# YooSungHyun/RNNTransducer

Measured on AMD Instinct MI355X. Metric: utterances/sec, higher is better.
Workload: dtype f32

## Files before the change

### include/rnnt_hip.h

```cpp
#ifndef RNNT_HIP_H_
#define RNNT_HIP_H_

#include <stddef.h>
#include <stdint.h>

#ifdef __cplusplus
extern "C" {
#endif

#define RNNT_HIP_ABI_VERSION 4

#define RNNT_OK 0
#define RNNT_ERR_INVALID (-1)
#define RNNT_ERR_LAUNCH (-2)
#define RNNT_ERR_UNSUPPORTED (-3)
#define RNNT_ERR_TIMEOUT (-4)

int rnnt_hip_version(void);
const char* rnnt_hip_last_error(void);
int rnnt_hip_device_cus(void);

enum {
  RNNT_K_GEMM = 0,
  RNNT_K_LSTM_FWD = 1,
// ... 24 lines not shown
  const float* A;
  int64_t a_div, a_so, a_si, a_sk;
  int32_t a_mc;
  const int64_t* a_rowidx;
  const float* B;
  int64_t b_sn, b_sk;
  float* C;
  int64_t c_div, c_so, c_si;
  const float* bias;
  const float* aux;
  uint32_t flags;
  void* workspace;
  size_t workspace_bytes;
} rnnt_gemm_desc;

size_t rnnt_hip_gemm_workspace_bytes(int64_t M, int64_t N, int64_t K);
int rnnt_hip_gemm_f32(const rnnt_gemm_desc* d, void* stream);

size_t rnnt_hip_hp_bytes(int64_t rows, int64_t K);
int rnnt_hip_hp_split(const float* x, int64_t rows, int64_t K, int64_t ld, int32_t transpose, int64_t src_rows, int64_t shift,
                      void* planes, uint32_t* amax, int32_t amax_given, void* stream);
int rnnt_hip_hp_split_both(const float* x, int64_t M, int64_t C, int64_t ld, const uint32_t* rowmax, const uint32_t* colmax,
                           void* planes_rm, void* planes_t, void* stream);
size_t rnnt_hip_gemm_hp_workspace_bytes(int64_t M, int64_t N, int64_t K);
int rnnt_hip_gemm_hp(const void* A, const uint32_t* a_amax, const void* B, const uint32_t* b_amax, int64_t M, int64_t N, int64_t K,
                     float* C, int64_t ldc, const float* bias, uint32_t flags, void* workspace, size_t workspace_bytes,
                     void* stream);

typedef struct rnnt_hp_problem {
  const void* A; const uint32_t* a_amax;
  const void* B; const uint32_t* b_amax;
  int64_t M, N, K;
  float* C; int64_t ldc;
  uint32_t flags;
} rnnt_hp_problem;
size_t rnnt_hip_gemm_hp_grouped_workspace_bytes(const rnnt_hp_problem* problems, int32_t n);
int rnnt_hip_gemm_hp_grouped(const rnnt_hp_problem* problems, int32_t n, uint32_t xcd_skip, void* workspace, size_t workspace_bytes,
                             void* stream);

#define RNNT_CELL_LSTM 0
#define RNNT_CELL_GRU 1
#define RNNT_CELL_RNN_TANH 2
#define RNNT_CELL_RNN_RELU 3

typedef struct rnnt_lstm_desc {
  int32_t T, B, I, H, D;
// ... 273 lines not shown
```

### rnntransducer_amd/_lib.py

```python
from __future__ import annotations

import ctypes as C
import os

_HERE = os.path.dirname(os.path.abspath(__file__))
LIB_PATH = os.environ.get("RNNT_HIP_LIB") or os.path.join(_HERE, "csrc", "librnnt_hip.so")
ABI_VERSION = 4

GEMM_GELU_A, GEMM_GELU_B, GEMM_ACCUM, GEMM_MUL_DGELU, GEMM_EXACT_F32 = 1, 2, 4, 8, 16
GEMM_HP_F16 = 32
PRECISION_FP32, PRECISION_F16 = 0, 1
CELL_LSTM, CELL_GRU, CELL_RNN_TANH, CELL_RNN_RELU = 0, 1, 2, 3

c_f32p = C.c_void_p
c_i64 = C.c_int64
c_i32 = C.c_int32


class GemmDesc(C.Structure):
    _fields_ = [("M", c_i64), ("N", c_i64), ("K", c_i64), ("A", C.c_void_p), ("a_div", c_i64), ("a_so", c_i64),
                ("a_si", c_i64), ("a_sk", c_i64), ("a_mc", c_i32), ("a_rowidx", C.c_void_p), ("B", C.c_void_p),
                ("b_sn", c_i64), ("b_sk", c_i64), ("C", C.c_void_p), ("c_div", c_i64), ("c_so", c_i64),
                ("c_si", c_i64), ("bias", C.c_void_p), ("aux", C.c_void_p), ("flags", C.c_uint32),
                ("workspace", C.c_void_p), ("workspace_bytes", C.c_size_t)]
# ... 85 lines not shown
                ("blank", c_i32), ("beam", c_i32), ("improved", c_i32), ("state_beam", C.c_double), ("expand_beam", C.c_double),
                ("max_candidates", c_i32), ("max_pops", c_i32), ("max_states", c_i32), ("max_nodes", c_i32), ("max_len", c_i32),
                ("A", C.c_void_p), ("lens", C.c_void_p), ("emb", C.c_void_p),
                ("w_ih", C.c_void_p * DECODE_MAX_LAYERS), ("w_hh", C.c_void_p * DECODE_MAX_LAYERS),
                ("b_ih", C.c_void_p * DECODE_MAX_LAYERS), ("b_hh", C.c_void_p * DECODE_MAX_LAYERS),
                ("w_o", C.c_void_p), ("b_o", C.c_void_p), ("w_d", C.c_void_p), ("ld_d", c_i64),
                ("workspace", C.c_void_p), ("workspace_bytes", C.c_size_t), ("tokens", C.c_void_p), ("out_lens", C.c_void_p),
                ("scores", C.c_void_p), ("count", C.c_void_p), ("status", C.c_void_p), ("commit", C.c_void_p),
                ("ncommit", C.c_void_p), ("stats", C.c_void_p)]


SYMBOLS = {
    "rnnt_hip_version": (C.c_int, []),
    "rnnt_hip_last_error": (C.c_char_p, []),
    "rnnt_hip_device_cus": (C.c_int, []),
    "rnnt_hip_prof_enable": (C.c_int, [C.c_int]),
    "rnnt_hip_prof_collect": (C.c_int, [C.c_void_p, C.c_void_p, C.c_void_p, C.c_int]),
    "rnnt_hip_lstm_launch_log_enable": (C.c_int, [C.c_int]),
    "rnnt_hip_lstm_launch_log": (c_i64, [C.c_char_p, C.c_size_t]),
    "rnnt_hip_gemm_workspace_bytes": (C.c_size_t, [c_i64, c_i64, c_i64]),
    "rnnt_hip_gemm_f32": (C.c_int, [C.POINTER(GemmDesc), C.c_void_p]),
    "rnnt_hip_hp_bytes": (C.c_size_t, [c_i64, c_i64]),
    "rnnt_hip_hp_split": (C.c_int, [C.c_void_p, c_i64, c_i64, c_i64, c_i32, c_i64, c_i64, C.c_void_p, C.c_void_p, c_i32, C.c_void_p]),
    "rnnt_hip_gemm_hp_workspace_bytes": (C.c_size_t, [c_i64, c_i64, c_i64]),
    "rnnt_hip_gemm_hp": (C.c_int, [C.c_void_p, C.c_void_p, C.c_void_p, C.c_void_p, c_i64, c_i64, c_i64, C.c_void_p, c_i64, C.c_void_p,
                                  C.c_uint32, C.c_void_p, C.c_size_t, C.c_void_p]),
    "rnnt_hip_hp_split_both": (C.c_int, [C.c_void_p, c_i64, c_i64, c_i64, C.c_void_p, C.c_void_p, C.c_void_p, C.c_void_p, C.c_void_p]),
    "rnnt_hip_gemm_hp_grouped_workspace_bytes": (C.c_size_t, [C.POINTER(HpProblem), c_i32]),
    "rnnt_hip_gemm_hp_grouped": (C.c_int, [C.POINTER(HpProblem), c_i32, C.c_uint32, C.c_void_p, C.c_size_t, C.c_void_p]),
    "rnnt_hip_lstm_workspace_bytes": (C.c_size_t, [c_i32] * 5),
    "rnnt_hip_lstm_max_batch": (c_i32, [c_i32, c_i32, c_i32]),
    "rnnt_hip_lstm_free_xcds": (c_i32, [c_i32] * 5),
    "rnnt_hip_lstm_takes_row_idx": (c_i32, [c_i32] * 6),
    "rnnt_hip_lstm_fwd": (C.c_int, [C.POINTER(LstmDesc), C.c_void_p]),
    "rnnt_hip_lstm_fwd_ex": (C.c_int, [C.POINTER(LstmDesc), C.c_uint32, C.c_void_p]),
    "rnnt_hip_lstm_takes_f16": (c_i32, [c_i32] * 6),
    "rnnt_hip_lstm_bwd": (C.c_int, [C.POINTER(LstmBwdDesc), C.c_void_p]),
    "rnnt_hip_lstm_bwd_ex": (C.c_int, [C.POINTER(LstmBwdDesc), C.c_uint32, C.c_void_p]),
    "rnnt_hip_lstm_check": (C.c_int, [C.c_void_p, C.c_void_p]),
    "rnnt_hip_lstm_debug_read": (C.c_int, [C.c_void_p, c_i32, c_i32, c_i32, c_i32, c_i32, C.c_void_p, c_i32, C.c_void_p]),
    "rnnt_hip_joint_loss_workspace_bytes": (C.c_size_t, [c_i32] * 4),
    "rnnt_hip_joint_loss_fwd_bwd": (C.c_int, [C.c_void_p, c_i64, c_i64, C.c_void_p, c_i64, c_i64, C.c_void_p, C.c_void_p,
                                               C.c_void_p, C.c_void_p, c_i32, c_i32, c_i32, c_i32, c_i32, C.c_float,
                                               C.c_void_p, C.c_void_p, C.c_void_p, C.c_void_p, C.c_size_t, C.c_void_p]),
    "rnnt_hip_joint_loss_bwd": (C.c_int, [C.c_void_p, c_i64, c_i64, C.c_void_p, c_i64, c_i64, C.c_void_p, C.c_void_p,
                                           C.c_void_p, C.c_void_p, c_i32, c_i32, c_i32, c_i32, c_i32, C.c_float, C.c_void_p, c_i32,
# ... 71 lines not shown
```

### rnntransducer_amd/csrc/common.hpp

```cpp
#pragma once
#include <hip/hip_runtime.h>
#include <stdarg.h>
#include <stdint.h>
#include <stdio.h>

#include <atomic>

#include "rnnt_hip.h"

namespace rnnt {

void set_error(const char* fmt, ...);

#define RNNT_CHECK_ARG(cond, ...)      \
  do {                                 \
    if (!(cond)) {                     \
      ::rnnt::set_error(__VA_ARGS__);  \
      return RNNT_ERR_INVALID;         \
    }                                  \
  } while (0)

#define RNNT_CHECK_HIP(expr)                                                          \
  do {                                                                                \
    hipError_t e_ = (expr);                                                           \
// ... 4 lines not shown
  } while (0)

#define RNNT_CHECK_LAUNCH() RNNT_CHECK_HIP(hipGetLastError())

struct ProfScope {
  ProfScope(int kind, double work, hipStream_t s);
  ~ProfScope();
  int kind_;
  double work_;
  hipStream_t stream_;
  void* start_;
};

extern std::atomic<bool> g_launch_log_on;
void launch_log_note(const void* kernel, hipStream_t s);

static inline int64_t ceil_div(int64_t a, int64_t b) { return (a + b - 1) / b; }

size_t hp_plane_bytes(int64_t rows, int64_t K);
int hp_colmax(const float* x, int64_t rows, int64_t C, int64_t ld, uint32_t* amax, hipStream_t s);
int hp_split(const float* x, int64_t rows, int64_t K, int64_t ld, uint32_t* amax, void* planes, hipStream_t s, const int* rowidx = nullptr);
int hp_split_t(const float* x, int64_t R, int64_t K, int64_t ld, int64_t Ksrc, int64_t shift, const uint32_t* amax, void* planes,
               hipStream_t s, const int* kidx = nullptr);
int hp_split_both(const float* x, int64_t M, int64_t C, int64_t ld, const uint32_t* rowmax, const uint32_t* colmax, void* planes_rm,
                  void* planes_t, hipStream_t s, const int* rowidx = nullptr);
size_t hp_gemm_workspace_bytes(int64_t M, int64_t N, int64_t K);
int hp_gemm(const void* A, const uint32_t* a_amax, const void* B, const uint32_t* b_amax, int64_t M, int64_t N, int64_t K, float* C,
            int64_t c_div, int64_t c_so, int64_t c_si, const float* bias, unsigned flags, void* workspace, size_t workspace_bytes,
            hipStream_t s, const int* a_rowidx = nullptr, int64_t a_plane_rows = 0, const int* c_rowidx = nullptr);
struct HpProblem {
  const void* A; const uint32_t* a_amax; const void* B; const uint32_t* b_amax;
  int64_t M, N, K;
  float* C; int64_t ldc;
  unsigned flags;
};
constexpr int HP_GROUP_MAX = 4;
size_t hp_gemm_grouped_workspace_bytes(const int64_t* MN, int n);
int hp_gemm_grouped(const HpProblem* pr, int n, unsigned xcd_skip, unsigned* counter, void* workspace, size_t workspace_bytes,
                    hipStream_t s, unsigned* status = nullptr);
constexpr size_t HPQ_HEADER_BYTES = 256;
static inline size_t align_up(size_t a, size_t b) { return (a + b - 1) / b * b; }

__device__ __forceinline__ float gelu_tanh(float x) {
  const float k0 = 0.7978845608028654f, k1 = 0.044715f;
  float u = k0 * (x + k1 * x * x * x);
  return 0.5f * x * (1.0f + tanhf(u));
// ... 51 lines not shown
```

### rnntransducer_amd/csrc/gemm_hp.hip

```cpp
#include "common.hpp"

#include <stdlib.h>

namespace rnnt {
namespace {

typedef _Float16 f16x8 __attribute__((ext_vector_type(8)));
typedef __attribute__((address_space(3))) void lds_void;

constexpr int HP_BM = 256, HP_BN = 256, HP_BK = 32;
constexpr int HP_STAGE = (HP_BM + HP_BN) * 128;
constexpr int HP_RSRC = 0x00027000;

__device__ __forceinline__ float hp_scale_from_amax(unsigned amax_bits) {
  int eb = (int)((amax_bits >> 23) & 255u);
  if (eb == 0) return 1.0f;
  eb = eb < 15 ? 15 : eb;
  return __uint_as_float((unsigned)(268 - eb) << 23);
}
__device__ __forceinline__ float hp_inv_scale_from_amax(unsigned amax_bits) {
  int eb = (int)((amax_bits >> 23) & 255u);
  if (eb == 0) return 1.0f;
  eb = eb < 15 ? 15 : eb;
  return __uint_as_float((unsigned)(eb - 14) << 23);
}

__global__ void __launch_bounds__(256) hp_colmax_kernel(const float* __restrict__ x, long rows, int C, long ld, long rows_per_chunk,
                                                        unsigned* __restrict__ out) {
  const int c = blockIdx.x * 256 + threadIdx.x;
  if (c >= C) return;
  const long r0 = (long)blockIdx.y * rows_per_chunk, r1 = min(rows, r0 + rows_per_chunk);
  unsigned m = 0;
  for (long r = r0; r < r1; ++r) m = max(m, __float_as_uint(x[r * ld + c]) & 0x7fffffffu);
  if (m != 0) atomicMax(out + c, m);
}

__device__ __forceinline__ void hp_split8(const float (&x)[8], float scale, u32x4& hi, u32x4& lo) {
  f16x8 h, l;
#pragma unroll
  for (int e = 0; e < 8; ++e) {
    const float v = x[e] * scale;
    const _Float16 a = (_Float16)v;
    h[e] = a;
    l[e] = (_Float16)(v - (float)a);
  }
  hi = __builtin_bit_cast(u32x4, h);
  lo = __builtin_bit_cast(u32x4, l);
}

__global__ void __launch_bounds__(256) hp_split_kernel(const float* __restrict__ x, long rows, int K, long ld, unsigned* __restrict__ amax,
                                                       char* __restrict__ out, const int* __restrict__ rowidx) {
  const int Kp = (K + 31) & ~31, cpr = Kp >> 3;
  const int lane = threadIdx.x & 63;
  const bool vec = (ld & 3) == 0 && (reinterpret_cast<uintptr_t>(x) & 15) == 0;
  for (long ri = (long)blockIdx.x * 4 + (threadIdx.x >> 6); ri < rows; ri += (long)gridDim.x * 4) {
    const long r = rowidx ? (long)rowidx[ri] : ri;
    const float* row = x + r * ld;
// ... 13 lines not shown
#pragma unroll
    for (int o = 32; o > 0; o >>= 1) m = max(m, (unsigned)__shfl_xor((int)m, o));
    if (lane == 0) amax[r] = m;
    const float scale = hp_scale_from_amax(m);
    for (int c = lane; c < cpr; c += 64) {
      const int k = 8 * c;
      float v[8];
      if (vec && k + 7 < K) {
        const f32x4 a = *reinterpret_cast<const f32x4*>(row + k), b = *reinterpret_cast<const f32x4*>(row + k + 4);
        v[0] = a[0]; v[1] = a[1]; v[2] = a[2]; v[3] = a[3]; v[4] = b[0]; v[5] = b[1]; v[6] = b[2]; v[7] = b[3];
      } else {
#pragma unroll
        for (int e = 0; e < 8; ++e) v[e] = (k + e < K) ? row[k + e] : 0.f;
      }
      u32x4 hi, lo;
      hp_split8(v, scale, hi, lo);
      char* dst = out + (r * (Kp >> 5) + (c >> 2)) * 128 + 16 * (c & 3);
      *reinterpret_cast<u32x4*>(dst) = hi;
      *reinterpret_cast<u32x4*>(dst + 64) = lo;
    }
  }
}

__global__ void __launch_bounds__(256) hp_split_t_kernel(const float* __restrict__ x, int R, int K, long ld, int Ksrc, int shift,
                                                         const unsigned* __restrict__ amax, char* __restrict__ out,
                                                         const int* __restrict__ kidx) {
  __shared__ float tile[32][257];
  const int kb = blockIdx.x, r0 = blockIdx.y * 256;
  const int tid = threadIdx.x;
  const bool vec = (ld & 3) == 0 && (reinterpret_cast<uintptr_t>(x) & 15) == 0;
#pragma unroll
  for (int q = 0; q < 8; ++q) {
    const int kk = 4 * q + (tid >> 6);
    const int kdst = kb * 32 + kk;
    const int ksrc = (kidx ? (kdst < K ? kidx[kdst] : 0) : kdst) + shift;
    const int c = 4 * (tid & 63);
    f32x4 v = {0.f, 0.f, 0.f, 0.f};
    if (kdst < K && ksrc >= 0 && ksrc < Ksrc) {
      const float* src = x + (long)ksrc * ld + r0 + c;
      if (vec && r0 + c + 3 < R) {
        v = *reinterpret_cast<const f32x4*>(src);
      } else {
#pragma unroll
        for (int e = 0; e < 4; ++e)
          if (r0 + c + e < R) v[e] = src[e];
      }
    }
#pragma unroll
    for (int e = 0; e < 4; ++e) tile[kk][c + e] = v[e];
  }
  __syncthreads();
  const int Kp32 = (K + 31) >> 5;
#pragma unroll
  for (int ps = 0; ps < 4; ++ps) {
    const int rl = (tid >> 2) + 64 * ps, ch = tid & 3;
    if (r0 + rl < R) {
      float v[8];
#pragma unroll
      for (int e = 0; e < 8; ++e) v[e] = tile[8 * ch + e][rl];
      u32x4 hi, lo;
      hp_split8(v, hp_scale_from_amax(amax[r0 + rl]), hi, lo);
      char* dst = out + ((long)(r0 + rl) * Kp32 + kb) * 128 + 16 * ch;
// ... 285 lines not shown
    counter[9] = 1u;
    if (status) __hip_atomic_store(status, 2u, __ATOMIC_RELAXED, __HIP_MEMORY_SCOPE_AGENT);
  }
}

__global__ void __launch_bounds__(256) hp_splitk_reduce_kernel(const HpGemmK p) {
  const long total = (long)p.M * p.N;
  for (long i = (long)blockIdx.x * 256 + threadIdx.x; i < total; i += (long)gridDim.x * 256) {
    const int m = (int)(i / p.N), n = (int)(i % p.N);
    float s = 0.f;
    for (int z = 0; z < p.splits; ++z) s += p.slab[(long)z * total + i];
    if (p.bias) s += p.bias[n];
    const int mo = p.c_rowidx ? p.c_rowidx[m] : m;
    const long off = (long)(mo / p.c_div) * p.c_so + (long)(mo % p.c_div) * p.c_si + n;
    if (p.flags & RNNT_GEMM_ACCUM) s += p.C[off];
    p.C[off] = s;
  }
}

}

size_t hp_plane_bytes(int64_t rows, int64_t K) { return (size_t)rows * (size_t)ceil_div(K, 32) * 128; }

int hp_colmax(const float* x, int64_t rows, int64_t C, int64_t ld, uint32_t* amax, hipStream_t s) {
  RNNT_CHECK_HIP(hipMemsetAsync(amax, 0, (size_t)C * 4, s));
  if (rows == 0 || C == 0) return RNNT_OK;
  long chunks = ceil_div(2048, ceil_div(C, 256));
  if (chunks > ceil_div(rows, 64)) chunks = ceil_div(rows, 64);
  if (chunks < 1) chunks = 1;
  const long rpc = ceil_div(rows, chunks);
  ProfScope prof(RNNT_K_HP_SPLIT, 4.0 * (double)rows * (double)C, s);
  hipLaunchKernelGGL(hp_colmax_kernel, dim3((unsigned)ceil_div(C, 256), (unsigned)ceil_div(rows, rpc)), dim3(256), 0, s, x, (long)rows, (int)C,
                     (long)ld, rpc, amax);
  RNNT_CHECK_LAUNCH();
  return RNNT_OK;
}

int hp_split(const float* x, int64_t rows, int64_t K, int64_t ld, uint32_t* amax, void* planes, hipStream_t s, const int* rowidx) {
  if (rows == 0) return RNNT_OK;
  const long blocks = ceil_div(rows, 4);
  ProfScope prof(RNNT_K_HP_SPLIT, 8.0 * (double)rows * (double)K, s);
  hipLaunchKernelGGL(hp_split_kernel, dim3((unsigned)(blocks < 8192 ? blocks : 8192)), dim3(256), 0, s, x, (long)rows, (int)K, (long)ld, amax,
                     (char*)planes, rowidx);
  RNNT_CHECK_LAUNCH();
  return RNNT_OK;
}

int hp_split_t(const float* x, int64_t R, int64_t K, int64_t ld, int64_t Ksrc, int64_t shift, const uint32_t* amax, void* planes,
               hipStream_t s, const int* kidx) {
  if (R == 0 || K == 0) return RNNT_OK;
  ProfScope prof(RNNT_K_HP_SPLIT, 8.0 * (double)R * (double)K, s);
  hipLaunchKernelGGL(hp_split_t_kernel, dim3((unsigned)ceil_div(K, 32), (unsigned)ceil_div(R, 256)), dim3(256), 0, s, x, (int)R, (int)K, (long)ld,
                     (int)Ksrc, (int)shift, amax, (char*)planes, kidx);
  RNNT_CHECK_LAUNCH();
  return RNNT_OK;
}

int hp_split_both(const float* x, int64_t M, int64_t C, int64_t ld, const uint32_t* rowmax, const uint32_t* colmax, void* planes_rm,
                  void* planes_t, hipStream_t s, const int* rowidx) {
  if (M == 0 || C == 0) return RNNT_OK;
  ProfScope prof(RNNT_K_HP_SPLIT, 12.0 * (double)M * (double)C, s);
  hipLaunchKernelGGL(hp_split_both_kernel, dim3((unsigned)ceil_div(M, 32), (unsigned)ceil_div(C, 256)), dim3(256), 0, s, x, (int)M, (int)C, (long)ld,
                     rowmax, colmax, (char*)planes_rm, (char*)planes_t, rowidx);
  RNNT_CHECK_LAUNCH();
  return RNNT_OK;
}

size_t hp_gemm_workspace_bytes(int64_t M, int64_t N, int64_t K) {
  const long tiles = ceil_div(M, HP_BM) * ceil_div(N, HP_BN);
  const long nkt = ceil_div(K, HP_BK);
  if (tiles >= 192 || nkt < 64) return 0;
  long want = ceil_div(256, tiles);
  if (want > nkt / 32) want = nkt / 32;
  if (want > 32) want = 32;
  return want >= 2 ? (size_t)want * M * N * 4 : 0;
}
// ... 16 lines not shown
  k.C = C; k.c_div = (int)(c_div > 0x7fffffff ? 0x7fffffff : c_div); k.c_so = c_so; k.c_si = c_si;
  k.bias = bias; k.flags = flags;
  k.a_rowidx = a_rowidx; k.c_rowidx = c_rowidx;
  const bool f16 = (flags & RNNT_GEMM_HP_F16) != 0u;
  k.tiles_m = (int)ceil_div(M, HP_BM); k.tiles_n = (int)ceil_div(N, HP_BN);
  const int tiles = k.tiles_m * k.tiles_n;
  {
    static const int env_gm = getenv("RNNT_GEMM_HP_GROUP_M") ? atoi(getenv("RNNT_GEMM_HP_GROUP_M")) : -1;
    k.group_m = env_gm >= 0 ? env_gm : (tiles >= 256 ? 8 : 4);
  }
  int splits = 1;
  if (workspace && tiles < 192 && k.nkt >= 64) {
    long want = ceil_div(256, tiles);
    const long by_ws = (long)(workspace_bytes / ((size_t)M * N * 4));
    if (want > k.nkt / 32) want = k.nkt / 32;
    if (want > by_ws) want = by_ws;
    if (want > 32) want = 32;
    if (want >= 2) splits = (int)want;
  }
  k.kt_per_split = (int)ceil_div(k.nkt, splits);
  splits = (int)ceil_div(k.nkt, k.kt_per_split);
  k.splits = splits;
  k.slab = (float*)workspace;
  if (f16) RNNT_CHECK_HIP(hipFuncSetAttribute((const void*)gemm_hp_kernel<true>, hipFuncAttributeMaxDynamicSharedMemorySize, 2 * HP_STAGE));
  else RNNT_CHECK_HIP(hipFuncSetAttribute((const void*)gemm_hp_kernel<false>, hipFuncAttributeMaxDynamicSharedMemorySize, 2 * HP_STAGE));
  {
    ProfScope prof(RNNT_K_GEMM_HP, 2.0 * (double)M * (double)N * (double)K, s);
    if (f16) hipLaunchKernelGGL(gemm_hp_kernel<true>, dim3(tiles, splits), dim3(512), 2 * HP_STAGE, s, k);
    else hipLaunchKernelGGL(gemm_hp_kernel<false>, dim3(tiles, splits), dim3(512), 2 * HP_STAGE, s, k);
    RNNT_CHECK_LAUNCH();
    if (splits > 1) {
      const long blocks = ceil_div((long)M * N, 256);
      hipLaunchKernelGGL(hp_splitk_reduce_kernel, dim3((unsigned)(blocks < 2048 ? blocks : 2048)), dim3(256), 0, s, k);
      RNNT_CHECK_LAUNCH();
    }
  }
  return RNNT_OK;
}

constexpr int HPQ_SPLIT_CAP = 8;
size_t hp_gemm_grouped_workspace_bytes(const int64_t* MN, int n) {
  size_t total = 0;
  for (int i = 0; i < n; ++i) total += align_up((size_t)HPQ_SPLIT_CAP * (size_t)MN[i] * 4, 256);
  return total;
}

int hp_gemm_grouped(const HpProblem* pr, int n, unsigned xcd_skip, unsigned* counter, void* workspace, size_t workspace_bytes,
                    hipStream_t s, unsigned* status) {
// ... 28 lines not shown
    k.tiles_m = (int)ceil_div(a.M, HP_BM); k.tiles_n = (int)ceil_div(a.N, HP_BN);
    total_kt += (long)k.tiles_m * k.tiles_n * k.nkt;
    flops += 2.0 * (double)a.M * (double)a.N * (double)a.K;
  }
  long chunk = ceil_div(total_kt, 4 * workers);
  if (chunk < 32) chunk = 32;
  size_t off = 0;
  int units = 0;
  for (int i = 0; i < n; ++i) {
    HpGemmK& k = q.prob[i];
    long splits = ceil_div(k.nkt, chunk);
    if (splits > HPQ_SPLIT_CAP) splits = HPQ_SPLIT_CAP;
    const size_t per = (size_t)k.M * k.N * 4;
    while (splits > 1 && (!workspace || off + align_up((size_t)splits * per, 256) > workspace_bytes)) --splits;
    k.kt_per_split = (int)ceil_div(k.nkt, splits);
    k.splits = (int)ceil_div(k.nkt, k.kt_per_split);
    k.slab = k.splits > 1 ? reinterpret_cast<float*>((char*)workspace + off) : nullptr;
    if (k.splits > 1) off += align_up((size_t)k.splits * per, 256);
    units += k.tiles_m * k.tiles_n * k.splits;
    q.unit_end[i] = units;
  }
  RNNT_CHECK_HIP(hipMemsetAsync(counter, 0, 64, s));
  const int lds = 2 * HP_STAGE + 16;
  const void* qk = f16 ? (const void*)gemm_hpq_kernel<true> : (const void*)gemm_hpq_kernel<false>;
  RNNT_CHECK_HIP(hipFuncSetAttribute(qk, hipFuncAttributeMaxDynamicSharedMemorySize, lds));
  {
    ProfScope prof(RNNT_K_GEMM_HP, flops, s);
    int cus = 0, dev = 0;
    if (hipGetDevice(&dev) != hipSuccess || hipDeviceGetAttribute(&cus, hipDeviceAttributeMultiprocessorCount, dev) != hipSuccess || cus < 8) cus = 256;
    const dim3 grid(!xcd_skip && units < cus ? units : cus);
    if (f16) hipLaunchKernelGGL(gemm_hpq_kernel<true>, grid, dim3(512), lds, s, q);
    else hipLaunchKernelGGL(gemm_hpq_kernel<false>, grid, dim3(512), lds, s, q);
    RNNT_CHECK_LAUNCH();
    hipLaunchKernelGGL(hpq_check_kernel, dim3(1), dim3(1), 0, s, counter, (unsigned)units, status);
    RNNT_CHECK_LAUNCH();
    for (int i = 0; i < n; ++i)
      if (q.prob[i].splits > 1) {
        const long blocks = ceil_div((long)q.prob[i].M * q.prob[i].N, 256);
        hipLaunchKernelGGL(hp_splitk_reduce_kernel, dim3((unsigned)(blocks < 2048 ? blocks : 2048)), dim3(256), 0, s, q.prob[i]);
        RNNT_CHECK_LAUNCH();
      }
  }
  return RNNT_OK;
}

}

using namespace rnnt;

extern "C" size_t rnnt_hip_hp_bytes(int64_t rows, int64_t K) {
  if (rows < 0 || K < 0) return 0;
  return hp_plane_bytes(rows, K);
}

extern "C" int rnnt_hip_hp_split(const float* x, int64_t rows, int64_t K, int64_t ld, int32_t transpose, int64_t src_rows, int64_t shift,
                                 void* planes, uint32_t* amax, int32_t amax_given, void* stream) {
  RNNT_CHECK_ARG(x && planes && amax && rows >= 0 && K >= 0, "hp_split: bad arguments");
  RNNT_CHECK_ARG((reinterpret_cast<uintptr_t>(planes) & 127) == 0, "hp_split: planes must be 128-byte aligned");
  hipStream_t s = (hipStream_t)stream;
  if (!transpose) {
    RNNT_CHECK_ARG(ld >= K, "hp_split: ld < K");
    RNNT_CHECK_ARG(!amax_given, "hp_split: the row-major split computes its row maxima itself");
    return hp_split(x, rows, K, ld, amax, planes, s);
  }
  RNNT_CHECK_ARG(ld >= rows && src_rows >= 1, "hp_split: transposed source is (src_rows x >= rows), ld >= rows");
  if (!amax_given)
    if (int rc = hp_colmax(x, src_rows, rows, ld, amax, s)) return rc;
  return hp_split_t(x, rows, K, ld, src_rows, shift, amax, planes, s);
}

extern "C" size_t rnnt_hip_gemm_hp_workspace_bytes(int64_t M, int64_t N, int64_t K) {
  if (M < 1 || N < 1 || K < 1) return 0;
  return hp_gemm_workspace_bytes(M, N, K);
}

extern "C" int rnnt_hip_gemm_hp(const void* A, const uint32_t* a_amax, const void* B, const uint32_t* b_amax, int64_t M, int64_t N,
                                int64_t K, float* C, int64_t ldc, const float* bias, uint32_t flags, void* workspace,
                                size_t workspace_bytes, void* stream) {
  RNNT_CHECK_ARG(ldc >= N, "gemm_hp: ldc < N");
  return hp_gemm(A, a_amax, B, b_amax, M, N, K, C, 1, ldc, 0, bias, flags, workspace, workspace_bytes, (hipStream_t)stream);
}

static_assert(sizeof(rnnt_hp_problem) == sizeof(HpProblem), "rnnt_hp_problem mirrors HpProblem");

extern "C" size_t rnnt_hip_gemm_hp_grouped_workspace_bytes(const rnnt_hp_problem* problems, int32_t n) {
  if (!problems || n < 1 || n > HP_GROUP_MAX) return 0;
  int64_t mn[HP_GROUP_MAX];
  for (int i = 0; i < n; ++i) mn[i] = problems[i].M * problems[i].N;
  return 256 + hp_gemm_grouped_workspace_bytes(mn, n);
}

extern "C" int rnnt_hip_gemm_hp_grouped(const rnnt_hp_problem* problems, int32_t n, uint32_t xcd_skip, void* workspace,
                                        size_t workspace_bytes, void* stream) {
// ... 20 lines not shown
```

### rnntransducer_amd/csrc/lstm.hip

```cpp
#include "lstm_shared.hpp"

#include <string.h>

namespace rnnt {
namespace {

template <int MT, int NT>
__global__ void __launch_bounds__(256) lstm_fwd_kernel(const LstmK p) {
  extern __shared__ __attribute__((aligned(16))) char smem[];
  float* Wl = reinterpret_cast<float*>(smem);
  f32x4* part = reinterpret_cast<f32x4*>(Wl + 4 * p.Hs * p.LDW);
  int* abort_lds = reinterpret_cast<int*>(part + 4 * MT * NT * 64);

  const int tid = threadIdx.x, lane = tid & 63, wave = tid >> 6;
  const int n = lane & 15, q = lane >> 4;
  const int d = blockIdx.x / p.NC, wg = blockIdx.x % p.NC;
  const int H = p.H, B = p.B, D = p.D, T = p.T, Bp = p.Bp, LDW = p.LDW;
  const int j0 = wg * p.Hs;
  const int R = 4 * p.Hs;

  {
    const float* W = p.w_hh[d];
    for (int idx = tid; idx < R * LDW; idx += 256) {
      const int r = idx / LDW, k = idx % LDW;
// ... 1801 lines not shown
  if (rc) return rc;

  const int64_t M = (int64_t)T * B, N4 = (int64_t)D * 4 * H;
  const int64_t Mv = ragged ? d->n_rows : M;
  const bool hp_in = w.hp && I >= 128;
  uint32_t* a_dgr = w.hp ? w.hp_amax + M + N4 : nullptr;
  uint32_t* a_dgc = w.hp ? a_dgr + M : nullptr;
  uint32_t* a_w = w.hp ? a_dgc + N4 : nullptr;
  uint32_t* a_x = w.hp ? a_w + I : nullptr;
  uint32_t* a_y = w.hp ? a_x + I : nullptr;
  if (w.hp) {
    const bool both = rowmax_done && colmax_done && hp_in && bd->dx;
    if (do_recur && hp_in && bd->dx) {
      if (both) rc = hp_split_both(d->gates, Mv, N4, N4, a_dgr, a_dgc, w.hp_dg, w.hp_dgt, s, ridx);
      else rc = hp_split(d->gates, Mv, N4, N4, a_dgr, w.hp_dg, s, ridx);
      if (rc) return rc;
    }
    if (do_weights && !colmax_done)
      if ((rc = hp_colmax(d->gates, M, N4, N4, a_dgc, s))) return rc;
    if (do_weights && !both)
      if ((rc = hp_split_t(d->gates, N4, Mv, N4, M, 0, a_dgc, w.hp_dgt, s, ridx))) return rc;
  }
  if (do_recur && bd->dx) {
    const long per = (long)4 * H * I;
    hipLaunchKernelGGL(permute_w_kernel, dim3((unsigned)ceil_div(per, 256), D), dim3(256), 0, s, d->w_ih[0],
                       D > 1 ? d->w_ih[1] : d->w_ih[0], H, I, ngate, w.wp);
    RNNT_CHECK_LAUNCH();
    if (hp_in) {
      if ((rc = hp_colmax(w.wp, N4, I, I, a_w, s))) return rc;
      if ((rc = hp_split_t(w.wp, I, N4, I, N4, 0, a_w, w.hp_w, s))) return rc;
      if ((rc = hp_gemm(w.hp_dg, a_dgr, w.hp_w, a_w, Mv, I, N4, bd->dx, 1, I, 0, nullptr, hpf, nullptr, 0, s, ridx, M, ridx))) return rc;
    } else {
      rnnt_gemm_desc g = {};
      g.M = M; g.N = I; g.K = N4;
      g.A = d->gates; g.a_div = 1; g.a_so = N4; g.a_si = 0; g.a_sk = 1; g.a_mc = 0;
      g.B = w.wp; g.b_sn = 1; g.b_sk = I;
      g.C = bd->dx; g.c_div = 1; g.c_so = I; g.c_si = 0;
      if ((rc = rnnt_hip_gemm_f32(&g, s))) return rc;
    }
    if (ragged) {
      const long nrow = (long)T * B;
      hipLaunchKernelGGL(zero_padded_rows_kernel, dim3((unsigned)(ceil_div(nrow, 4) < 2048 ? ceil_div(nrow, 4) : 2048)), dim3(256), 0, s, bd->dx, d->lens, T, B, I);
      RNNT_CHECK_LAUNCH();
    }
  }
  if (!do_weights) return RNNT_OK;
  const bool grouped = w.hp && hp_in && T > 1 && !gru && D <= 2 && (xcd_skip != 0u || getenv("RNNT_GEMM_HP_GROUP")) && !getenv("RNNT_GEMM_HP_NO_GROUP");
  {
    const bool x_plain = d->x_sb == I && d->x_st == (int64_t)B * I;
    if (hp_in || (w.hp && I >= 32 && x_plain && !getenv("RNNT_GEMM_HP_NO_NARROW"))) {
      if (d->x_abs_bound > 0.f) {
        uint32_t bits;
        memcpy(&bits, &d->x_abs_bound, 4);
        RNNT_CHECK_HIP(hipMemsetD32Async((hipDeviceptr_t)a_x, (int)bits, (size_t)I, s));
      } else if ((rc = hp_colmax(d->x, M, I, I, a_x, s))) return rc;
// ... 8 lines not shown
      g.C = w.wp; g.c_div = 1; g.c_so = I; g.c_si = 0;
      g.workspace = w.scratch; g.workspace_bytes = w.scratch_bytes;
      if ((rc = rnnt_hip_gemm_f32(&g, s))) return rc;
    }
    if (!grouped) {
      const long per = (long)4 * H * I;
      hipLaunchKernelGGL(unpermute_w_kernel, dim3((unsigned)ceil_div(per, 256), D), dim3(256), 0, s, w.wp, H, I, per, ngate,
                         bd->dw_ih[0], D > 1 ? bd->dw_ih[1] : bd->dw_ih[0], acc);
      RNNT_CHECK_LAUNCH();
    }
  }
  if (w.hp && T > 1) {
    if (d->cell != RNNT_CELL_RNN_RELU) {
      RNNT_CHECK_HIP(hipMemsetD32Async((hipDeviceptr_t)a_y, 0x3f800000, (size_t)D * H, s));
    } else if ((rc = hp_colmax(d->y, M, (int64_t)D * H, (int64_t)D * H, a_y, s))) return rc;
    if (gru) {
      if (colmax_done) a_dgc = a_y + (int64_t)D * H;
      else if ((rc = hp_colmax(ghid, M, N4, N4, a_dgc, s))) return rc;
      if ((rc = hp_split_t(ghid, N4, Mv, N4, M, 0, a_dgc, w.hp_dgt, s, ridx))) return rc;
    }
    HpProblem pr[HP_GROUP_MAX];
    int npr = 0;
    if (grouped) pr[npr++] = HpProblem{w.hp_dgt, a_dgc, w.hp_x, a_x, N4, I, Mv, w.wp, I, hpf};
    for (int dir = 0; dir < D; ++dir) {
      char* yt = w.hp_yt + (size_t)dir * hp_plane_bytes(H, M);
      if ((rc = hp_split_t(d->y + (int64_t)dir * H, H, Mv, (int64_t)D * H, M, dir == 0 ? -B : B, a_y + (int64_t)dir * H, yt, s, ridx))) return rc;
      const char* ag = w.hp_dgt + (size_t)dir * 4 * H * (size_t)ceil_div(Mv, 32) * 128;
      if (grouped) {
        pr[npr++] = HpProblem{ag, a_dgc + (int64_t)dir * 4 * H, yt, a_y + (int64_t)dir * H, 4 * H, H, Mv, w.dwhh + (int64_t)dir * 4 * H * H, H, hpf};
        continue;
      }
      if ((rc = hp_gemm(ag, a_dgc + (int64_t)dir * 4 * H, yt, a_y + (int64_t)dir * H, 4 * H, H, Mv, w.dwhh + (int64_t)dir * 4 * H * H, 1, H, 0,
                        nullptr, hpf, w.scratch, w.scratch_bytes, s)))
        return rc;
    }
    if (grouped) {
      if ((rc = hp_gemm_grouped(pr, npr, xcd_skip, reinterpret_cast<unsigned*>(w.scratch), (char*)w.scratch + HPQ_HEADER_BYTES,
                                w.scratch_bytes - HPQ_HEADER_BYTES, s, k.status)))
        return rc;
      const long per = (long)4 * H * I;
      hipLaunchKernelGGL(unpermute_w_kernel, dim3((unsigned)ceil_div(per, 256), D), dim3(256), 0, s, w.wp, H, I, per, ngate,
                         bd->dw_ih[0], D > 1 ? bd->dw_ih[1] : bd->dw_ih[0], acc);
      RNNT_CHECK_LAUNCH();
    }
  } else
  for (int dir = 0; dir < D; ++dir) {
    rnnt_gemm_desc g = {};
    g.M = 4 * H; g.N = H; g.K = (int64_t)(T - 1) * B;
    const int64_t shift_g = dir == 0 ? (int64_t)B * N4 : 0;
// ... 117 lines not shown
```

Before: 1296.

## Fuse weight permute into split-t kernel and batch per-direction plane splits

Drops the separate permute_w kernel in the high-precision backward path: a new weight-planes function reads the original per-direction input weights directly, computing the gate permutation inside the transposed split kernel. The colmax kernel is vectorised with a shared-memory reduction and can process both directions in one launch. Per-direction y splits are batched into a single launch using the grid z dimension, and hipFuncSetAttribute calls are cached in function-local statics. These changes aim to cut launch count and a full intermediate weight write/read, at the cost of more index math per element and extra code paths.

```diff
diff --git a/include/rnnt_hip.h b/include/rnnt_hip.h
--- a/include/rnnt_hip.h
+++ b/include/rnnt_hip.h
@@ -70,6 +70,10 @@
                       void* planes, uint32_t* amax, int32_t amax_given, void* stream);
 int rnnt_hip_hp_split_both(const float* x, int64_t M, int64_t C, int64_t ld, const uint32_t* rowmax, const uint32_t* colmax,
                            void* planes_rm, void* planes_t, void* stream);
+int rnnt_hip_hp_split_t_batch(const float* const* x, const int64_t* shift, const uint32_t* const* amax, void* const* planes, int32_t n,
+                              int64_t rows, int64_t K, int64_t ld, int64_t src_rows, const int32_t* kidx, void* stream);
+int rnnt_hip_hp_weight_planes_t(const float* w0, const float* w1, int32_t D, int32_t H, int64_t I, int32_t ngate, void* planes,
+                                uint32_t* amax, void* stream);
 size_t rnnt_hip_gemm_hp_workspace_bytes(int64_t M, int64_t N, int64_t K);
 int rnnt_hip_gemm_hp(const void* A, const uint32_t* a_amax, const void* B, const uint32_t* b_amax, int64_t M, int64_t N, int64_t K,
                      float* C, int64_t ldc, const float* bias, uint32_t flags, void* workspace, size_t workspace_bytes,
diff --git a/rnntransducer_amd/_lib.py b/rnntransducer_amd/_lib.py
--- a/rnntransducer_amd/_lib.py
+++ b/rnntransducer_amd/_lib.py
@@ -131,6 +131,9 @@
     "rnnt_hip_gemm_f32": (C.c_int, [C.POINTER(GemmDesc), C.c_void_p]),
     "rnnt_hip_hp_bytes": (C.c_size_t, [c_i64, c_i64]),
     "rnnt_hip_hp_split": (C.c_int, [C.c_void_p, c_i64, c_i64, c_i64, c_i32, c_i64, c_i64, C.c_void_p, C.c_void_p, c_i32, C.c_void_p]),
+    "rnnt_hip_hp_split_t_batch": (C.c_int, [C.c_void_p, C.c_void_p, C.c_void_p, C.c_void_p, c_i32, c_i64, c_i64, c_i64, c_i64, C.c_void_p,
+                                           C.c_void_p]),
+    "rnnt_hip_hp_weight_planes_t": (C.c_int, [C.c_void_p, C.c_void_p, c_i32, c_i32, c_i64, c_i32, C.c_void_p, C.c_void_p, C.c_void_p]),
     "rnnt_hip_gemm_hp_workspace_bytes": (C.c_size_t, [c_i64, c_i64, c_i64]),
     "rnnt_hip_gemm_hp": (C.c_int, [C.c_void_p, C.c_void_p, C.c_void_p, C.c_void_p, c_i64, c_i64, c_i64, C.c_void_p, c_i64, C.c_void_p,
                                   C.c_uint32, C.c_void_p, C.c_size_t, C.c_void_p]),
diff --git a/rnntransducer_amd/csrc/common.hpp b/rnntransducer_amd/csrc/common.hpp
--- a/rnntransducer_amd/csrc/common.hpp
+++ b/rnntransducer_amd/csrc/common.hpp
@@ -50,6 +50,10 @@
 int hp_split(const float* x, int64_t rows, int64_t K, int64_t ld, uint32_t* amax, void* planes, hipStream_t s, const int* rowidx = nullptr);
 int hp_split_t(const float* x, int64_t R, int64_t K, int64_t ld, int64_t Ksrc, int64_t shift, const uint32_t* amax, void* planes,
                hipStream_t s, const int* kidx = nullptr);
+struct HpSplitTItem { const float* x; const uint32_t* amax; void* planes; int64_t shift; };
+int hp_split_t_batch(const HpSplitTItem* items, int n, int64_t R, int64_t K, int64_t ld, int64_t Ksrc, hipStream_t s, const int* kidx = nullptr);
+int hp_weight_planes_t(const float* w0, const float* w1, int D, int64_t H, int64_t I, int ngate, uint32_t* amax, void* planes, bool amax_zeroed,
+                       hipStream_t s);
 int hp_split_both(const float* x, int64_t M, int64_t C, int64_t ld, const uint32_t* rowmax, const uint32_t* colmax, void* planes_rm,
                   void* planes_t, hipStream_t s, const int* rowidx = nullptr);
 size_t hp_gemm_workspace_bytes(int64_t M, int64_t N, int64_t K);
diff --git a/rnntransducer_amd/csrc/gemm_hp.hip b/rnntransducer_amd/csrc/gemm_hp.hip
--- a/rnntransducer_amd/csrc/gemm_hp.hip
+++ b/rnntransducer_amd/csrc/gemm_hp.hip
@@ -25,14 +25,33 @@
   return __uint_as_float((unsigned)(eb - 14) << 23);
 }
 
-__global__ void __launch_bounds__(256) hp_colmax_kernel(const float* __restrict__ x, long rows, int C, long ld, long rows_per_chunk,
-                                                        unsigned* __restrict__ out) {
-  const int c = blockIdx.x * 256 + threadIdx.x;
-  if (c >= C) return;
+__global__ void __launch_bounds__(256) hp_colmax_kernel(const float* __restrict__ x0, const float* __restrict__ x1, long rows, int C, long ld,
+                                                        long rows_per_chunk, unsigned* __restrict__ out) {
+  __shared__ unsigned red[4][256];
+  const float* __restrict__ x = blockIdx.z ? x1 : x0;
+  const int tid = threadIdx.x, rl = tid >> 6, cl = 4 * (tid & 63);
+  const int c = blockIdx.x * 256 + cl;
   const long r0 = (long)blockIdx.y * rows_per_chunk, r1 = min(rows, r0 + rows_per_chunk);
-  unsigned m = 0;
-  for (long r = r0; r < r1; ++r) m = max(m, __float_as_uint(x[r * ld + c]) & 0x7fffffffu);
-  if (m != 0) atomicMax(out + c, m);
+  const bool vec = (ld & 3) == 0 && (reinterpret_cast<uintptr_t>(x) & 15) == 0 && c + 3 < C;
+  unsigned m[4] = {0u, 0u, 0u, 0u};
+  if (vec) {
+#pragma unroll 4
+    for (long r = r0 + rl; r < r1; r += 4) {
+      const u32x4 v = *reinterpret_cast<const u32x4*>(x + r * ld + c);
+#pragma unroll
+      for (int e = 0; e < 4; ++e) m[e] = max(m[e], v[e] & 0x7fffffffu);
+    }
+  } else {
+    for (long r = r0 + rl; r < r1; r += 4)
+#pragma unroll
+      for (int e = 0; e < 4; ++e)
+        if (c + e < C) m[e] = max(m[e], __float_as_uint(x[r * ld + c + e]) & 0x7fffffffu);
+  }
+#pragma unroll
+  for (int e = 0; e < 4; ++e) red[rl][cl + e] = m[e];
+  __syncthreads();
+  const unsigned mm = max(max(red[0][tid], red[1][tid]), max(red[2][tid], red[3][tid]));
+  if (mm != 0 && blockIdx.x * 256 + tid < C) atomicMax(out + blockIdx.x * 256 + tid, mm);
 }
 
 __device__ __forceinline__ void hp_split8(const float (&x)[8], float scale, u32x4& hi, u32x4& lo) {
@@ -92,22 +111,46 @@
   }
 }
 
-__global__ void __launch_bounds__(256) hp_split_t_kernel(const float* __restrict__ x, int R, int K, long ld, int Ksrc, int shift,
-                                                         const unsigned* __restrict__ amax, char* __restrict__ out,
-                                                         const int* __restrict__ kidx) {
+constexpr int HP_SPLIT_T_MAX = 2;
+struct HpSplitT {
+  const float* x[HP_SPLIT_T_MAX];
+  const unsigned* amax[HP_SPLIT_T_MAX];
+  char* out[HP_SPLIT_T_MAX];
+  int shift[HP_SPLIT_T_MAX];
+  int R, K, Ksrc;
+  long ld;
+  const int* kidx;
+  int perm_H, perm_ngate;
+};
+
+__global__ void __launch_bounds__(256) hp_split_t_kernel(const HpSplitT a) {
   __shared__ float tile[32][257];
   const int kb = blockIdx.x, r0 = blockIdx.y * 256;
   const int tid = threadIdx.x;
-  const bool vec = (ld & 3) == 0 && (reinterpret_cast<uintptr_t>(x) & 15) == 0;
+  const bool second = blockIdx.z != 0;
+  const int R = a.R, K = a.K;
+  const int shift = second ? a.shift[1] : a.shift[0];
+  const unsigned* __restrict__ amax = second ? a.amax[1] : a.amax[0];
+  char* __restrict__ out = second ? a.out[1] : a.out[0];
+  const bool vec = (a.ld & 3) == 0 && ((reinterpret_cast<uintptr_t>(a.x[0]) | reinterpret_cast<uintptr_t>(a.x[1])) & 15) == 0;
 #pragma unroll
   for (int q = 0; q < 8; ++q) {
     const int kk = 4 * q + (tid >> 6);
     const int kdst = kb * 32 + kk;
-    const int ksrc = (kidx ? (kdst < K ? kidx[kdst] : 0) : kdst) + shift;
+    const float* row = nullptr;
+    if (kdst < K) {
+      if (a.perm_H > 0) {
+        const int d = kdst / (4 * a.perm_H), r = kdst - d * 4 * a.perm_H, g = r & 3;
+        if (g < a.perm_ngate) row = (d ? a.x[1] : a.x[0]) + (long)(g * a.perm_H + (r >> 2)) * a.ld;
+      } else {
+        const int ksrc = (a.kidx ? a.kidx[kdst] : kdst) + shift;
+        if (ksrc >= 0 && ksrc < a.Ksrc) row = (second ? a.x[1] : a.x[0]) + (long)ksrc * a.ld;
+      }
+    }
     const int c = 4 * (tid & 63);
     f32x4 v = {0.f, 0.f, 0.f, 0.f};
-    if (kdst < K && ksrc >= 0 && ksrc < Ksrc) {
-      const float* src = x + (long)ksrc * ld + r0 + c;
+    if (row) {
+      const float* src = row + r0 + c;
       if (vec && r0 + c + 3 < R) {
         v = *reinterpret_cast<const f32x4*>(src);
       } else {
@@ -439,18 +482,22 @@
 
 size_t hp_plane_bytes(int64_t rows, int64_t K) { return (size_t)rows * (size_t)ceil_div(K, 32) * 128; }
 
-int hp_colmax(const float* x, int64_t rows, int64_t C, int64_t ld, uint32_t* amax, hipStream_t s) {
-  RNNT_CHECK_HIP(hipMemsetAsync(amax, 0, (size_t)C * 4, s));
+static int hp_colmax_launch(const float* x0, const float* x1, int nsrc, int64_t rows, int64_t C, int64_t ld, uint32_t* amax, hipStream_t s) {
   if (rows == 0 || C == 0) return RNNT_OK;
-  long chunks = ceil_div(2048, ceil_div(C, 256));
+  long chunks = ceil_div(2048, ceil_div(C, 256) * nsrc);
   if (chunks > ceil_div(rows, 64)) chunks = ceil_div(rows, 64);
   if (chunks < 1) chunks = 1;
   const long rpc = ceil_div(rows, chunks);
-  ProfScope prof(RNNT_K_HP_SPLIT, 4.0 * (double)rows * (double)C, s);
-  hipLaunchKernelGGL(hp_colmax_kernel, dim3((unsigned)ceil_div(C, 256), (unsigned)ceil_div(rows, rpc)), dim3(256), 0, s, x, (long)rows, (int)C,
-                     (long)ld, rpc, amax);
+  ProfScope prof(RNNT_K_HP_SPLIT, 4.0 * (double)rows * (double)C * nsrc, s);
+  hipLaunchKernelGGL(hp_colmax_kernel, dim3((unsigned)ceil_div(C, 256), (unsigned)ceil_div(rows, rpc), (unsigned)nsrc), dim3(256), 0, s, x0, x1,
+                     (long)rows, (int)C, (long)ld, rpc, amax);
   RNNT_CHECK_LAUNCH();
   return RNNT_OK;
+}
+
+int hp_colmax(const float* x, int64_t rows, int64_t C, int64_t ld, uint32_t* amax, hipStream_t s) {
+  RNNT_CHECK_HIP(hipMemsetAsync(amax, 0, (size_t)C * 4, s));
+  return hp_colmax_launch(x, x, 1, rows, C, ld, amax, s);
 }
 
 int hp_split(const float* x, int64_t rows, int64_t K, int64_t ld, uint32_t* amax, void* planes, hipStream_t s, const int* rowidx) {
@@ -463,12 +510,39 @@
   return RNNT_OK;
 }
 
+int hp_split_t_batch(const HpSplitTItem* it, int n, int64_t R, int64_t K, int64_t ld, int64_t Ksrc, hipStream_t s, const int* kidx) {
+  RNNT_CHECK_ARG(it && n >= 1 && n <= HP_SPLIT_T_MAX, "hp_split_t: 1..%d items", HP_SPLIT_T_MAX);
+  if (R == 0 || K == 0) return RNNT_OK;
+  HpSplitT a = {};
+  for (int i = 0; i < HP_SPLIT_T_MAX; ++i) {
+    const HpSplitTItem& j = it[i < n ? i : 0];
+    a.x[i] = j.x; a.amax[i] = j.amax; a.out[i] = (char*)j.planes; a.shift[i] = (int)j.shift;
+  }
+  a.R = (int)R; a.K = (int)K; a.Ksrc = (int)Ksrc; a.ld = (long)ld; a.kidx = kidx;
+  ProfScope prof(RNNT_K_HP_SPLIT, 8.0 * (double)R * (double)K * n, s);
+  hipLaunchKernelGGL(hp_split_t_kernel, dim3((unsigned)ceil_div(K, 32), (unsigned)ceil_div(R, 256), (unsigned)n), dim3(256), 0, s, a);
+  RNNT_CHECK_LAUNCH();
+  return RNNT_OK;
+}
+
 int hp_split_t(const float* x, int64_t R, int64_t K, int64_t ld, int64_t Ksrc, int64_t shift, const uint32_t* amax, void* planes,
                hipStream_t s, const int* kidx) {
-  if (R == 0 || K == 0) return RNNT_OK;
-  ProfScope prof(RNNT_K_HP_SPLIT, 8.0 * (double)R * (double)K, s);
-  hipLaunchKernelGGL(hp_split_t_kernel, dim3((unsigned)ceil_div(K, 32), (unsigned)ceil_div(R, 256)), dim3(256), 0, s, x, (int)R, (int)K, (long)ld,
-                     (int)Ksrc, (int)shift, amax, (char*)planes, kidx);
+  const HpSplitTItem it = {x, amax, planes, shift};
+  return hp_split_t_batch(&it, 1, R, K, ld, Ksrc, s, kidx);
+}
+
+int hp_weight_planes_t(const float* w0, const float* w1, int D, int64_t H, int64_t I, int ngate, uint32_t* amax, void* planes, bool amax_zeroed,
+                       hipStream_t s) {
+  RNNT_CHECK_ARG(w0 && (D == 1 || w1) && (D == 1 || D == 2) && H >= 1 && I >= 1 && ngate >= 1 && ngate <= 4, "hp_weight_planes_t: bad arguments");
+  if (!amax_zeroed) RNNT_CHECK_HIP(hipMemsetAsync(amax, 0, (size_t)I * 4, s));
+  if (int rc = hp_colmax_launch(w0, D > 1 ? w1 : w0, D, (int64_t)ngate * H, I, I, amax, s)) return rc;
+  HpSplitT a = {};
+  a.x[0] = w0; a.x[1] = D > 1 ? w1 : w0;
+  a.amax[0] = a.amax[1] = amax; a.out[0] = a.out[1] = (char*)planes;
+  a.R = (int)I; a.K = (int)(D * 4 * H); a.Ksrc = a.K; a.ld = (long)I;
+  a.perm_H = (int)H; a.perm_ngate = ngate;
+  ProfScope prof(RNNT_K_HP_SPLIT, 8.0 * (double)a.R * (double)a.K, s);
+  hipLaunchKernelGGL(hp_split_t_kernel, dim3((unsigned)ceil_div(a.K, 32), (unsigned)ceil_div(I, 256), 1u), dim3(256), 0, s, a);
   RNNT_CHECK_LAUNCH();
   return RNNT_OK;
 }
@@ -531,8 +605,13 @@
   splits = (int)ceil_div(k.nkt, k.kt_per_split);
   k.splits = splits;
   k.slab = (float*)workspace;
-  if (f16) RNNT_CHECK_HIP(hipFuncSetAttribute((const void*)gemm_hp_kernel<true>, hipFuncAttributeMaxDynamicSharedMemorySize, 2 * HP_STAGE));
-  else RNNT_CHECK_HIP(hipFuncSetAttribute((const void*)gemm_hp_kernel<false>, hipFuncAttributeMaxDynamicSharedMemorySize, 2 * HP_STAGE));
+  {
+    static const hipError_t lds_ok = [] {
+      const hipError_t e = hipFuncSetAttribute((const void*)gemm_hp_kernel<true>, hipFuncAttributeMaxDynamicSharedMemorySize, 2 * HP_STAGE);
+      return e != hipSuccess ? e : hipFuncSetAttribute((const void*)gemm_hp_kernel<false>, hipFuncAttributeMaxDynamicSharedMemorySize, 2 * HP_STAGE);
+    }();
+    RNNT_CHECK_HIP(lds_ok);
+  }
   {
     ProfScope prof(RNNT_K_GEMM_HP, 2.0 * (double)M * (double)N * (double)K, s);
     if (f16) hipLaunchKernelGGL(gemm_hp_kernel<true>, dim3(tiles, splits), dim3(512), 2 * HP_STAGE, s, k);
@@ -607,8 +686,13 @@
   }
   RNNT_CHECK_HIP(hipMemsetAsync(counter, 0, 64, s));
   const int lds = 2 * HP_STAGE + 16;
-  const void* qk = f16 ? (const void*)gemm_hpq_kernel<true> : (const void*)gemm_hpq_kernel<false>;
-  RNNT_CHECK_HIP(hipFuncSetAttribute(qk, hipFuncAttributeMaxDynamicSharedMemorySize, lds));
+  {
+    static const hipError_t lds_ok = [] {
+      const hipError_t e = hipFuncSetAttribute((const void*)gemm_hpq_kernel<true>, hipFuncAttributeMaxDynamicSharedMemorySize, 2 * HP_STAGE + 16);
+      return e != hipSuccess ? e : hipFuncSetAttribute((const void*)gemm_hpq_kernel<false>, hipFuncAttributeMaxDynamicSharedMemorySize, 2 * HP_STAGE + 16);
+    }();
+    RNNT_CHECK_HIP(lds_ok);
+  }
   {
     ProfScope prof(RNNT_K_GEMM_HP, flops, s);
     int cus = 0, dev = 0;
@@ -654,6 +738,27 @@
   return hp_split_t(x, rows, K, ld, src_rows, shift, amax, planes, s);
 }
 
+extern "C" int rnnt_hip_hp_split_t_batch(const float* const* x, const int64_t* shift, const uint32_t* const* amax, void* const* planes, int32_t n,
+                                         int64_t rows, int64_t K, int64_t ld, int64_t src_rows, const int32_t* kidx, void* stream) {
+  RNNT_CHECK_ARG(x && shift && amax && planes && n >= 1 && n <= HP_SPLIT_T_MAX, "hp_split_t_batch: 1..%d items", HP_SPLIT_T_MAX);
+  RNNT_CHECK_ARG(rows >= 0 && K >= 0 && ld >= rows && src_rows >= 1 && rows < (1ll << 31) && K < (1ll << 31) && src_rows < (1ll << 31),
+                 "hp_split_t_batch: the sources are (src_rows x >= rows) views, ld >= rows");
+  HpSplitTItem it[HP_SPLIT_T_MAX];
+  for (int i = 0; i < n; ++i) {
+    RNNT_CHECK_ARG(x[i] && amax[i] && planes[i] && (reinterpret_cast<uintptr_t>(planes[i]) & 127) == 0,
+                   "hp_split_t_batch: item %d needs a source, its maxima and 128-byte aligned planes", i);
+    it[i] = HpSplitTItem{x[i], amax[i], planes[i], shift[i]};
+  }
+  return hp_split_t_batch(it, n, rows, K, ld, src_rows, (hipStream_t)stream, kidx);
+}
+
+extern "C" int rnnt_hip_hp_weight_planes_t(const float* w0, const float* w1, int32_t D, int32_t H, int64_t I, int32_t ngate, void* planes,
+                                           uint32_t* amax, void* stream) {
+  RNNT_CHECK_ARG(planes && amax && (reinterpret_cast<uintptr_t>(planes) & 127) == 0, "hp_weight_planes_t: planes (128-byte aligned) and amax");
+  RNNT_CHECK_ARG(I < (1ll << 31) && (int64_t)D * 4 * H < (1ll << 31), "hp_weight_planes_t: dims must fit 31 bits");
+  return hp_weight_planes_t(w0, w1, D, H, I, ngate, amax, planes, false, (hipStream_t)stream);
+}
+
 extern "C" size_t rnnt_hip_gemm_hp_workspace_bytes(int64_t M, int64_t N, int64_t K) {
   if (M < 1 || N < 1 || K < 1) return 0;
   return hp_gemm_workspace_bytes(M, N, K);
diff --git a/rnntransducer_amd/csrc/lstm.hip b/rnntransducer_amd/csrc/lstm.hip
--- a/rnntransducer_amd/csrc/lstm.hip
+++ b/rnntransducer_amd/csrc/lstm.hip
@@ -1847,15 +1847,14 @@
       if ((rc = hp_split_t(d->gates, N4, Mv, N4, M, 0, a_dgc, w.hp_dgt, s, ridx))) return rc;
   }
   if (do_recur && bd->dx) {
-    const long per = (long)4 * H * I;
-    hipLaunchKernelGGL(permute_w_kernel, dim3((unsigned)ceil_div(per, 256), D), dim3(256), 0, s, d->w_ih[0],
-                       D > 1 ? d->w_ih[1] : d->w_ih[0], H, I, ngate, w.wp);
-    RNNT_CHECK_LAUNCH();
     if (hp_in) {
-      if ((rc = hp_colmax(w.wp, N4, I, I, a_w, s))) return rc;
-      if ((rc = hp_split_t(w.wp, I, N4, I, N4, 0, a_w, w.hp_w, s))) return rc;
+      if ((rc = hp_weight_planes_t(d->w_ih[0], D > 1 ? d->w_ih[1] : d->w_ih[0], D, H, I, ngate, a_w, w.hp_w, colmax_done, s))) return rc;
       if ((rc = hp_gemm(w.hp_dg, a_dgr, w.hp_w, a_w, Mv, I, N4, bd->dx, 1, I, 0, nullptr, hpf, nullptr, 0, s, ridx, M, ridx))) return rc;
     } else {
+      const long per = (long)4 * H * I;
+      hipLaunchKernelGGL(permute_w_kernel, dim3((unsigned)ceil_div(per, 256), D), dim3(256), 0, s, d->w_ih[0],
+                         D > 1 ? d->w_ih[1] : d->w_ih[0], H, I, ngate, w.wp);
+      RNNT_CHECK_LAUNCH();
       rnnt_gemm_desc g = {};
       g.M = M; g.N = I; g.K = N4;
       g.A = d->gates; g.a_div = 1; g.a_so = N4; g.a_si = 0; g.a_sk = 1; g.a_mc = 0;
@@ -1910,9 +1909,14 @@
     HpProblem pr[HP_GROUP_MAX];
     int npr = 0;
     if (grouped) pr[npr++] = HpProblem{w.hp_dgt, a_dgc, w.hp_x, a_x, N4, I, Mv, w.wp, I, hpf};
+    {
+      HpSplitTItem it[2];
+      for (int dir = 0; dir < D; ++dir)
+        it[dir] = HpSplitTItem{d->y + (int64_t)dir * H, a_y + (int64_t)dir * H, w.hp_yt + (size_t)dir * hp_plane_bytes(H, M), dir == 0 ? -B : B};
+      if ((rc = hp_split_t_batch(it, D, H, Mv, (int64_t)D * H, M, s, ridx))) return rc;
+    }
     for (int dir = 0; dir < D; ++dir) {
       char* yt = w.hp_yt + (size_t)dir * hp_plane_bytes(H, M);
-      if ((rc = hp_split_t(d->y + (int64_t)dir * H, H, Mv, (int64_t)D * H, M, dir == 0 ? -B : B, a_y + (int64_t)dir * H, yt, s, ridx))) return rc;
       const char* ag = w.hp_dgt + (size_t)dir * 4 * H * (size_t)ceil_div(Mv, 32) * 128;
       if (grouped) {
         pr[npr++] = HpProblem{ag, a_dgc + (int64_t)dir * 4 * H, yt, a_y + (int64_t)dir * H, 4 * H, H, Mv, w.dwhh + (int64_t)dir * 4 * H * H, H, hpf};
```

Result: no change. 1302 (median of 6 runs) (+0.5%).
